# veronicaguerrini/LiME

Measured on AMD Instinct MI355X. Metric: eBWT symbols/s processed (ClusterLCP+ClusterBWT_DA), higher is better.
Workload: dtype u8

## Files before the change

include/lime_hip.h:

```cpp
#ifndef LIME_HIP_H
#define LIME_HIP_H
#include <stddef.h>
#include <stdint.h>

#ifdef __cplusplus
extern "C" {
#endif

#define LIME_OK            0
#define LIME_ERR_ARG      (-1)
#define LIME_ERR_HIP      (-2)
#define LIME_ERR_NOMEM    (-3)
#define LIME_ERR_MAXLEN   (-4)
#define LIME_ERR_HALO     (-5)
#define LIME_ERR_DOCID    (-6)
#define LIME_ERR_IO       (-7)

#define LIME_MAX_CLUSTER  65536u
#define LIME_TILE         4096u
#define LIME_FASTA_BLOCK  4096u

typedef struct lime_ctx lime_ctx;

typedef struct { uint64_t pStart, len; } lime_cluster_t;
// ... 78 lines not shown
                   const uint8_t *d_ebwt, uint64_t n_own, uint64_t n_avail, int eof,
                   uint32_t n_reads, uint32_t n_refs, uint32_t alpha,
                   uint8_t *d_sim, int zero_sim, void *stream);

typedef struct {
    uint32_t n_bins, bin_shift;
    const uint32_t *d_recs;
    const uint64_t *d_binbase;
    const uint64_t *d_bigrecs;
    uint64_t n_bigrecs;
} lime_records_t;
int lime_records_layout(lime_ctx *ctx, uint32_t n_reads, uint32_t n_refs, uint32_t *n_bins, uint32_t *bin_shift);
int lime_fused_records_dev(lime_ctx *ctx, const uint32_t *d_lcp, const uint32_t *d_da, const uint8_t *d_ebwt,
                           uint64_t n_own, uint64_t n_avail, int eof, uint32_t n_reads, uint32_t n_refs,
                           uint32_t alpha, void *stream);
int lime_records_get(lime_ctx *ctx, lime_records_t *out, uint64_t *h_binbase , void *stream);
int lime_apply_records_dev(lime_ctx *ctx, uint32_t n_src, const uint32_t *d_rx, const uint64_t *h_srcoff ,
                           uint32_t nb, uint32_t bin_shift, const uint64_t *d_bigrecs, uint64_t n_bigrecs,
                           uint64_t cell_lo, uint64_t block_bytes, uint8_t *d_block, void *stream);

int lime_partition_records_dev(lime_ctx *ctx, uint32_t n_prod, uint32_t prod_waves, uint32_t n_sub, uint32_t cap_w, const uint32_t *h_pool,
                               const uint32_t *h_wave_cnt, uint32_t n_bins, uint32_t bin_shift, uint32_t *d_out, uint64_t out_words,
                               uint64_t *h_binbase , int *kernel , void *stream);

int lime_combine_edges(const uint32_t *edge, uint32_t n_shards);

int lime_detect_dev(lime_ctx *ctx, const uint32_t *d_lcp, const uint32_t *d_da,
                    uint64_t n_own, uint64_t n_avail, int eof, uint64_t pos_base,
                    uint32_t n_reads, uint32_t alpha,
                    const lime_cluster_t **d_clusters, uint64_t *n_clusters, uint64_t *max_len,
                    void *stream);

int lime_score_dev(lime_ctx *ctx, const uint32_t *d_da, const uint8_t *d_ebwt, uint64_t n,
                   const lime_cluster_t *d_clusters, uint64_t n_clusters,
                   uint32_t n_reads, uint32_t n_refs, uint8_t *d_sim, int zero_sim, void *stream);

int lime_choose_dev(lime_ctx *ctx, const uint8_t *d_sim, uint32_t n_reads, uint32_t n_refs,
                    uint8_t *d_row_max, uint32_t *d_row_nnz, void *stream);

int lime_choose_pairs_dev(lime_ctx *ctx, const uint8_t *d_sim, uint32_t n_reads, uint32_t n_refs,
                          uint32_t norm, float beta, uint8_t *row_max, uint64_t *row_off,
                          lime_pair_t **pairs, uint64_t *n_pairs, void *stream);

int lime_fused_choose_dev(lime_ctx *ctx, const uint32_t *d_lcp, const uint32_t *d_da, const uint8_t *d_ebwt, uint64_t n,
                          uint32_t n_reads, uint32_t n_refs, uint32_t alpha, uint32_t norm, float beta,
                          uint8_t *row_max, uint64_t *row_off, lime_pair_t **pairs, uint64_t *n_pairs,
// ... 23 lines not shown
int  lime_comm_exchange_records(lime_comm *comm, lime_ctx *ctx, uint32_t n_reads, uint32_t n_refs, uint8_t *d_block,
                                size_t block_cap, uint64_t *cell_lo, uint64_t *block_bytes, void *stream);

int  lime_fused_multi(int n_dev, const int *devices, const uint32_t *lcp, const uint32_t *da, const uint8_t *ebwt,
                      uint64_t n, uint32_t n_reads, uint32_t n_refs, uint32_t alpha, uint8_t *sim,
                      uint64_t *n_clusters, uint64_t *max_len);

int  lime_score_choose_multi(int n_dev, const int *devices, const uint32_t *da, const uint8_t *ebwt, uint64_t n,
                             const lime_cluster_t *clusters, uint64_t n_clusters, uint32_t n_reads, uint32_t n_refs,
                             uint32_t norm, float beta, uint8_t *row_max, uint64_t *row_off, lime_pair_t **pairs,
                             uint64_t *n_pairs);

uint8_t lime_sym_index(uint8_t byte);
uint8_t lime_pair_score(const uint8_t cr[16], const uint8_t cg[16]);

typedef struct { uint32_t n_bins, bin_shift, n_sub, sub_rb, sub_gb; } lime_rec_layout_t;
int      lime_rec_layout(uint32_t n_reads, uint32_t n_refs, uint32_t one_level, uint32_t two_level, lime_rec_layout_t *out);
int      lime_rec_valid(uint32_t gd, uint32_t n_refs);
uint32_t lime_rec_of(uint32_t rd, uint32_t gd, uint32_t n_refs);
uint32_t lime_rec_sub2(uint32_t rd, uint32_t gd, uint32_t sub_rb, uint32_t sub_gb);
uint32_t lime_rec_bin(uint32_t rec, uint32_t sub, uint32_t bin_shift);
int      lime_rec_batch(const uint32_t *rd, const uint32_t *gd, uint64_t n, uint32_t n_refs, const lime_rec_layout_t *layout,
                        int fixed_slot, uint8_t *valid, uint8_t *stored, uint32_t *rec, uint32_t *sub, uint32_t *bin);
typedef struct { uint32_t cap, cap_short, room_left, top_left; } lime_scan_queue_t;
void     lime_scan_queue(lime_scan_queue_t *out);

int lime_write_clrs(const char *path, const lime_cluster_t *clusters, uint64_t n_clusters);
int lime_write_aux(const char *path, uint32_t n_reads, uint32_t n_refs, uint32_t alpha,
                   uint64_t max_len, uint64_t n_clusters);
int lime_read_aux(const char *path, uint32_t *n_reads, uint32_t *n_refs, uint32_t *alpha,
                  uint64_t *max_len, uint64_t *n_clusters);
int lime_write_res_txt(const char *path, const uint8_t *sim, const uint8_t *row_max,
                       uint32_t n_reads, uint32_t n_refs, uint32_t norm, float beta);
int lime_write_res_bin(const char *path_bin, const char *path_pos, const uint8_t *sim,
                       const uint8_t *row_max, uint32_t n_reads, uint32_t n_refs,
                       uint32_t norm, float beta);
int lime_write_res_txt_pairs(const char *path, const uint8_t *row_max, const uint64_t *row_off,
                             const lime_pair_t *pairs, uint32_t n_reads, uint32_t norm, float beta);
int lime_write_res_bin_pairs(const char *path_bin, const char *path_pos, const uint8_t *row_max,
                             const uint64_t *row_off, const lime_pair_t *pairs, uint32_t n_reads,
                             uint32_t norm, float beta);

int lime_classify(uint32_t n_files, const char *const *inputs, int binary, uint32_t n_reads,
                  uint32_t n_targ, const char *path_out, const char *path_tax, int rank, int higher,
                  uint64_t counts[4]);
const char *lime_classify_error(void);
// ... 168 lines not shown
```

lime_amd/_lib.py:

```python
from __future__ import annotations

import ctypes as C
import os

_DIR = os.path.dirname(os.path.abspath(__file__))
LIB_PATH = os.environ.get("LIME_LIB") or os.path.join(_DIR, "liblime_hip.so")

LIME_OK = 0
ERR_ARG, ERR_HIP, ERR_NOMEM, ERR_MAXLEN, ERR_HALO, ERR_DOCID, ERR_IO = -1, -2, -3, -4, -5, -6, -7
MAX_CLUSTER = 65536
TILE = 4096
FASTA_BLOCK = 4096


class Cluster(C.Structure):
    _fields_ = [("pStart", C.c_uint64), ("len", C.c_uint64)]


class Stats(C.Structure):
    _fields_ = [("n_clusters", C.c_uint64), ("max_len", C.c_uint64), ("n_updates", C.c_uint64),
                ("n_cross", C.c_uint32), ("n_big", C.c_uint32), ("flags", C.c_uint32), ("wave_records_max", C.c_uint32), ("edge", C.c_uint32), ("reserved", C.c_uint32)]


class Records(C.Structure):
# ... 48 lines not shown
    "lime_register_file": (_i, [_vp, _sz, _i]),
    "lime_unregister_file": (None, [_vp]),
    "lime_score": (_i, [_vp, _vp, _vp, _u64, _vp, _u64, _u32, _u32, _vp]),
    "lime_fused": (_i, [_vp, _vp, _vp, _vp, _u64, _u32, _u32, _u32, _vp, _pu64, _pu64]),
    "lime_choose": (_i, [_vp, _vp, _u32, _u32, _vp, _vp]),
    "lime_sim_bytes": (_sz, [_u32, _u32]),
    "lime_fused_dev": (_i, [_vp, _vp, _vp, _vp, _u64, _u64, _i, _u32, _u32, _u32, _vp, _i, _vp]),
    "lime_detect_dev": (_i, [_vp, _vp, _vp, _u64, _u64, _i, _u64, _u32, _u32, _pp, _pu64, _pu64, _vp]),
    "lime_score_dev": (_i, [_vp, _vp, _vp, _u64, _vp, _u64, _u32, _u32, _vp, _i, _vp]),
    "lime_choose_dev": (_i, [_vp, _vp, _u32, _u32, _vp, _vp, _vp]),
    "lime_synth_dev": (_i, [_vp, _u64, _u64, _u64, _u32, _u32, _u32, _u32, _vp, _vp, _vp, _vp]),
    "lime_get_stats": (_i, [_vp, C.POINTER(Stats), _vp]),
    "lime_set_timing": (_i, [_vp, _i]),
    "lime_get_timing": (_i, [_vp, C.POINTER(C.c_double), _pu64]),
    "lime_get_timing_ex": (_i, [_vp, C.POINTER(C.c_double), _pu64]),
    "lime_get_host_times": (_i, [_vp, C.POINTER(C.c_double)]),
    "lime_sym_index": (C.c_uint8, [C.c_uint8]),
    "lime_pair_score": (C.c_uint8, [_vp, _vp]),
    "lime_rec_layout": (_i, [_u32, _u32, _u32, _u32, _vp]),
    "lime_rec_valid": (_i, [_u32, _u32]),
    "lime_rec_of": (_u32, [_u32, _u32, _u32]),
    "lime_rec_sub2": (_u32, [_u32, _u32, _u32, _u32]),
    "lime_rec_bin": (_u32, [_u32, _u32, _u32]),
    "lime_rec_batch": (_i, [_vp, _vp, _u64, _u32, _vp, _i, _vp, _vp, _vp, _vp, _vp]),
    "lime_scan_queue": (None, [_vp]),
    "lime_write_clrs": (_i, [C.c_char_p, _vp, _u64]),
    "lime_write_aux": (_i, [C.c_char_p, _u32, _u32, _u32, _u64, _u64]),
    "lime_read_aux": (_i, [C.c_char_p, C.POINTER(_u32), C.POINTER(_u32), C.POINTER(_u32), _pu64, _pu64]),
    "lime_write_res_txt": (_i, [C.c_char_p, _vp, _vp, _u32, _u32, _u32, C.c_float]),
    "lime_write_res_bin": (_i, [C.c_char_p, C.c_char_p, _vp, _vp, _u32, _u32, _u32, C.c_float]),
    "lime_classify": (_i, [_u32, _vp, _i, _u32, _u32, C.c_char_p, C.c_char_p, _i, _i, _vp]),
    "lime_classify_error": (C.c_char_p, []),
    "lime_fused_stream": (_i, [_vp, _vp, _vp, _vp, _u64, _u32, _u32, _u32, _u64, _vp, _pu64, _pu64]),
    "lime_choose_pairs_dev": (_i, [_vp, _vp, _u32, _u32, _u32, C.c_float, _vp, _vp, _pp, _pu64, _vp]),
    "lime_fused_choose_dev": (_i, [_vp, _vp, _vp, _vp, _u64, _u32, _u32, _u32, _u32, C.c_float, _vp, _vp, _pp, _pu64, C.POINTER(Stats), _vp]),
    "lime_score_choose": (_i, [_vp, _vp, _vp, _u64, _vp, _u64, _u32, _u32, _u32, C.c_float, _vp, _vp, _pp, _pu64, _vp]),
    "lime_combine_edges": (_i, [_vp, _u32]),
    "lime_comm_unique_id": (_i, [_vp]),
    "lime_comm_init": (_i, [_vp, _i, _i, _pp]),
    "lime_comm_destroy": (None, [_vp]),
    "lime_comm_count": (_i, [_vp, C.POINTER(_i)]),
    "lime_comm_error": (C.c_char_p, []),
    "lime_comm_reduce_scatter_tables": (_i, [_vp, _vp, _vp, _sz, _vp]),
    "lime_comm_allreduce_tables": (_i, [_vp, _vp, _sz, _vp]),
    "lime_comm_combine_counters": (_i, [_vp, _vp, _vp]),
    "lime_records_layout": (_i, [_vp, _u32, _u32, C.POINTER(_u32), C.POINTER(_u32)]),
    "lime_fused_records_dev": (_i, [_vp, _vp, _vp, _vp, _u64, _u64, _i, _u32, _u32, _u32, _vp]),
    "lime_records_get": (_i, [_vp, _vp, _vp, _vp]),
    "lime_apply_records_dev": (_i, [_vp, _u32, _vp, _vp, _u32, _u32, _vp, _u64, _u64, _u64, _vp, _vp]),
    "lime_partition_records_dev": (_i, [_vp, _u32, _u32, _u32, _u32, _vp, _vp, _u32, _u32, _vp, _u64, _vp, C.POINTER(_i), _vp]),
    "lime_comm_exchange_records": (_i, [_vp, _vp, _u32, _u32, _vp, _sz, _pu64, _pu64, _vp]),
    "lime_fused_multi": (_i, [_i, _vp, _vp, _vp, _vp, _u64, _u32, _u32, _u32, _vp, _pu64, _pu64]),
    "lime_score_choose_multi": (_i, [_i, _vp, _vp, _vp, _u64, _vp, _u64, _u32, _u32, _u32, C.c_float, _vp, _vp, _pp, _pu64]),
    "lime_write_res_txt_pairs": (_i, [C.c_char_p, _vp, _vp, _vp, _u32, _u32, C.c_float]),
    "lime_write_res_bin_pairs": (_i, [C.c_char_p, C.c_char_p, _vp, _vp, _vp, _u32, _u32, C.c_float]),
    "lime_choose_lists_dev": (_i, [_vp, _vp, _u32, _u32, _u32, C.c_float, _pp, _vp]),
    "lime_fused_choose_lists_dev": (_i, [_vp, _vp, _vp, _vp, _u64, _u32, _u32, _u32, _u32, C.c_float, _pp, C.POINTER(Stats), _vp]),
    "lime_fused_choose_lists": (_i, [_vp, _vp, _vp, _vp, _u64, _u32, _u32, _u32, _u32, C.c_float, _pp, C.POINTER(Stats)]),
    "lime_lists_get": (_i, [_vp, _vp, _vp, _pp, _pu64]),
    "lime_lists_info": (_i, [_vp, C.POINTER(_u32), _pu64, C.POINTER(_u32), C.POINTER(C.c_float)]),
    "lime_lists_free": (None, [_vp]),
    "lime_lists_concat_dev": (_i, [_vp, _u32, _vp, _vp, _vp, C.c_float, _pp, _vp]),
    "lime_lists_concat_norms_dev": (_i, [_vp, _u32, _vp, _vp, _vp, _vp, C.c_float, _pp, _vp]),
    "lime_lists_get_norms": (_i, [_vp, _vp]),
    "lime_taxonomy_load": (_i, [C.c_char_p, _i, _i, _u32, _pp]),
    "lime_taxonomy_free": (None, [_vp]),
    "lime_classify_lists_dev": (_i, [_vp, _u32, _vp, _u32, _vp, _i, _vp, _vp, _vp]),
    "lime_classify_mem": (_i, [_u32, _vp, _vp, _vp, _vp, _vp, _i, _u32, _u32, _vp, _vp, _vp]),
    "lime_classify_mem_norms": (_i, [_u32, _vp, _vp, _vp, _vp, _vp, _vp, _i, _u32, _u32, _vp, _vp, _vp]),
    "lime_write_classification": (_i, [C.c_char_p, _vp, _u32]),
    "lime_index_size": (_u64, [_vp, _u32]),
    "lime_build_index": (_i, [_vp, _vp, _vp, _u32, C.c_uint8, _u32, _vp, _vp, _vp]),
# ... 114 lines not shown
```

lime_amd/api.py:

```python
from __future__ import annotations

import ctypes as C
import os

import numpy as np

from . import _lib
from ._lib import Cluster, LimeError, Stats, check, check_cls

FASTA_BLOCK = _lib.FASTA_BLOCK
NORM_PER_READ = 0xFFFFFFFF
VERDICT = np.dtype([("taxon", "<u4"), ("sim", "<f4"), ("type", "u1"), ("rule", "u1"), ("pad", "u1", (2,))])


class _LibBuf:
    def __init__(self, lib, ptr, words):
        self._lib, self._ptr = lib, ptr
        self.__array_interface__ = {"data": (ptr, False), "shape": (words,), "typestr": "<u4", "version": 3}

    def __del__(self):
        try:
            self._lib.lime_free(C.c_void_p(self._ptr))
        except Exception:
            pass
# ... 209 lines not shown
        nb, sh = C.c_uint32(0), C.c_uint32(0)
        check(self.lib.lime_records_layout(self.h, n_reads, n_refs, C.byref(nb), C.byref(sh)))
        return int(nb.value), int(sh.value)

    def fused_records_dev(self, lcp_t, da_t, ebwt_t, n_own, n_avail, eof, n_reads, n_refs, alpha, stream=None):
        self._rec_shape = self.records_layout(n_reads, n_refs)
        check(self.lib.lime_fused_records_dev(self.h, _ptr(lcp_t), _ptr(da_t), _ptr(ebwt_t), n_own, n_avail, int(eof),
                                              n_reads, n_refs, alpha, stream))

    def records_get(self, stream=None):
        import numpy as np
        from ._lib import Records
        nb, _ = self._rec_shape
        r = Records()
        base = np.zeros(nb + 1, dtype=np.uint64)
        check(self.lib.lime_records_get(self.h, C.byref(r), base.ctypes.data, stream))
        return r, base

    def apply_records_dev(self, n_src, rx_t, srcoff, nb, bin_shift, bigrecs_t, n_big, cell_lo, block_bytes, block_t, stream=None):
        import numpy as np
        so = np.ascontiguousarray(srcoff, dtype=np.uint64)
        check(self.lib.lime_apply_records_dev(self.h, n_src, _ptr(rx_t), so.ctypes.data, nb, bin_shift, _ptr(bigrecs_t), n_big,
                                              cell_lo, block_bytes, _ptr(block_t), stream))

    def partition_records(self, n_prod, prod_waves, n_sub, cap_w, pool, wave_cnt, n_bins, bin_shift, out_t, out_words=None, stream=None):
        import numpy as np
        pool = np.ascontiguousarray(pool, dtype=np.uint32)
        wc = np.ascontiguousarray(wave_cnt, dtype=np.uint32)
        base = np.zeros(n_bins + 1, dtype=np.uint64)
        kernel = C.c_int(-1)
        check(self.lib.lime_partition_records_dev(self.h, n_prod, prod_waves, n_sub, cap_w, pool.ctypes.data, wc.ctypes.data, n_bins, bin_shift,
                                                  _ptr(out_t), out_t.numel() if out_words is None else out_words, base.ctypes.data,
                                                  C.byref(kernel), stream))
        return base, int(kernel.value)

    def detect_dev(self, lcp_t, da_t, n_own, n_avail, eof, pos_base, n_reads, alpha, stream=None):
        dc, nc, ml = C.c_void_p(), C.c_uint64(0), C.c_uint64(0)
        check(self.lib.lime_detect_dev(self.h, _ptr(lcp_t), _ptr(da_t), n_own, n_avail, int(eof), pos_base, n_reads,
                                       alpha, C.byref(dc), C.byref(nc), C.byref(ml), stream))
        return dc.value, int(nc.value), int(ml.value)

    def score_dev(self, da_t, ebwt_t, n, clusters_ptr, n_clusters, n_reads, n_refs, sim_t, zero_sim=True, stream=None):
        check(self.lib.lime_score_dev(self.h, _ptr(da_t), _ptr(ebwt_t), n, C.c_void_p(clusters_ptr), n_clusters, n_reads,
                                      n_refs, _ptr(sim_t), int(zero_sim), stream))

    def choose_dev(self, sim_t, n_reads, n_refs, max_t, nnz_t, stream=None):
# ... 1126 lines not shown
```

lime_amd/csrc/lime_api.cpp:

```cpp
#include <hip/hip_runtime.h>
#include <stdarg.h>
#include <stdio.h>
#include <stdlib.h>
#include <string.h>
#include <memory>
#include <string>
#include <vector>

#include "lime_device.h"
#include "lime_ctx.h"

using namespace lime;
using namespace lime_host;

static thread_local std::string g_err;

int lime_host::fail(int code, const char *fmt, ...)
{
    char buf[512];
    va_list ap; va_start(ap, fmt); vsnprintf(buf, sizeof buf, fmt, ap); va_end(ap);
    g_err = buf;
    return code;
}

// ... 308 lines not shown

extern "C" uint8_t lime_pair_score(const uint8_t cr[16], const uint8_t cg[16])
{
    uint32_t r[4] = {0, 0, 0, 0}, g[4] = {0, 0, 0, 0};
    for (int i = 0; i < 16; ++i) { r[i >> 2] |= (uint32_t)cr[i] << ((i & 3) * 8); g[i >> 2] |= (uint32_t)cg[i] << ((i & 3) * 8); }
    return (uint8_t)pair_score(r, g);
}

extern "C" int lime_rec_layout(uint32_t n_reads, uint32_t n_refs, uint32_t one_level, uint32_t two_level, lime_rec_layout_t *out)
{
    if (!n_reads || !n_refs || !out) return fail(LIME_ERR_ARG, "lime_rec_layout: bad argument");
    const size_t sim_bytes = lime_sim_bytes(n_reads, n_refs);
    if (sim_bytes > ((size_t)BIN_MAX << BIN_SHIFT_MAX) || sim_bytes >= (1ull << CELL_BITS) || sim_bytes > ((uint64_t)MAX_SUB << 32))
        return fail(LIME_ERR_ARG, "lime_rec_layout: table too large for update records");
    const bool forced = one_level && two_level;
    bin_layout_of(forced ? one_level : BIN_ONE_LEVEL, forced ? two_level : BIN_TWO_LEVEL, forced, sim_bytes, &out->n_bins, &out->bin_shift);
    sub_layout(sim_bytes, n_refs, &out->n_sub, &out->sub_rb, &out->sub_gb);
    return LIME_OK;
}
extern "C" int lime_rec_valid(uint32_t gd, uint32_t n_refs) { return genome_ok(gd, n_refs) ? 1 : 0; }
extern "C" uint32_t lime_rec_of(uint32_t rd, uint32_t gd, uint32_t n_refs) { return rec_of(rd, gd, n_refs); }
extern "C" uint32_t lime_rec_sub2(uint32_t rd, uint32_t gd, uint32_t sub_rb, uint32_t sub_gb) { return rec_sub2(rd, gd, sub_rb, sub_gb); }
extern "C" uint32_t lime_rec_bin(uint32_t rec, uint32_t sub, uint32_t bin_shift) { return rec_bin(rec, sub, bin_shift); }
extern "C" void lime_scan_queue(lime_scan_queue_t *out)
{
    if (out) { out->cap = QCAP_SCAN; out->cap_short = QCAP_SCAN_SHORT; out->room_left = ROOM_LEFT; out->top_left = FLUSH_GRAN - 1u; }
}
extern "C" int lime_rec_batch(const uint32_t *rd, const uint32_t *gd, uint64_t n, uint32_t n_refs, const lime_rec_layout_t *lay, int fixed_slot,
                              uint8_t *valid, uint8_t *stored, uint32_t *rec, uint32_t *sub, uint32_t *bin)
{
    if (!lay || !n_refs || (n && (!rd || !gd || !valid || !stored || !rec || !sub || !bin))) return fail(LIME_ERR_ARG, "lime_rec_batch: bad argument");
    for (uint64_t i = 0; i < n; ++i) {
        valid[i] = genome_ok(gd[i], n_refs);
        stored[i] = rec_stored(rd[i], gd[i], n_refs, lay->n_sub, lay->sub_rb, lay->sub_gb, fixed_slot != 0, rec[i], sub[i]);
        bin[i] = rec_bin(rec[i], sub[i], lay->bin_shift);
    }
    return LIME_OK;
}
```

lime_amd/csrc/lime_apply.hip:

```cpp
#define LIME_DEBUG_TU_APPLY
#include <hip/hip_runtime.h>
#include <stdint.h>
#include <string.h>
#include <atomic>
#include "lime_device.h"
#include "lime_kernels.h"
#include "lime_wave.h"
#include "lime_debug.h"
#include "lime_launch.h"

namespace lime {

__device__ __forceinline__ uint32_t keep_bytes(uint32_t x, uint32_t wb, uint32_t s, uint32_t e)
{
    uint32_t m = 0xFFFFFFFFu;
    if (wb < s) { const uint32_t d = s - wb; m = d >= 4u ? 0u : m << (8u * d); }
    if (wb + 4u > e) { const uint32_t d = e > wb ? e - wb : 0u; m &= d >= 4u ? 0xFFFFFFFFu : ((1u << (8u * d)) - 1u); }
    return x & m;
}
__device__ __forceinline__ uint32_t nz_bytes(uint32_t x) { return (((x & 0x7F7F7F7Fu) + 0x7F7F7F7Fu) | x) & 0x80808080u; }

constexpr uint32_t FIN_SEGS = 258;
__device__ __forceinline__ void fin_region_store(uint32_t *seg_acc, const ApplyFin &f, uint32_t region, uint64_t r0, uint32_t o0, uint32_t nseg, uint32_t len)
{
// ... 252 lines not shown
            for (uint32_t q = cur.q + 2u * LG; __ballot(q * 4u < cur.fe); q += 2u * LG) {
                uint2 w0 = make_uint2(0u, 0u), w1 = make_uint2(0u, 0u);
                if (q * 4u < cur.fe) w0 = *reinterpret_cast<const uint2 *>(cur.src + (size_t)q * 4u);
                if ((q + 1u) * 4u < cur.fe) w1 = *reinterpret_cast<const uint2 *>(cur.src + (size_t)(q + 1u) * 4u);
                add4c(q * 4u < cur.fe, q * 4u, w0, cur.fa, cur.fe);
                add4c((q + 1u) * 4u < cur.fe, (q + 1u) * 4u, w1, cur.fa, cur.fe);
            }
        }
    };
    uint32_t region = (gridDim.x & 7u) ? blockIdx.x : (blockIdx.x & 7u) * (gridDim.x >> 3) + (blockIdx.x >> 3);
    if (region >= n_regions) return;
    uint32_t row0 = tbase[region >> bsh], n_rows = tbase[(region >> bsh) + 1u] - row0;
    uint32_t a, e;
    index_of(region, row0, n_rows, 0u, a, e);
    uint4 ri = make_uint4(0u, 0u, 0u, 0u);
    if (MODE != 0) ri = fin.region_rows[region];
    if (MODE == 1) for (uint32_t i = threadIdx.x; i < 2u * FIN_SEGS; i += APPLY_WG) seg_acc[i] = 0u;
    bool clean = false;
    __syncthreads();
    AP_DECL
    for (;;) {
        const uint32_t next = region + gridDim.x;
        const bool more = next < n_regions;
        uint32_t nrow0 = 0, nrow1 = 0;
        if (more) { nrow0 = tbase[next >> bsh]; nrow1 = tbase[(next >> bsh) + 1u]; }
        uint4 nri = make_uint4(0u, 0u, 0u, 0u);
        if (MODE != 0 && more) nri = fin.region_rows[next];
        const bool skip = MODE == 2 && (ri.w >> 31) != 0u;
        if (MODE == 1 && threadIdx.x == 0) qovf_s[par ^ 1u] = 0u;
        if (!skip)
        for (exact = false;; exact = true) {
        qn = 0u;
        if (!(MODE == 1 && clean && !exact)) {
            for (uint32_t i = threadIdx.x; i < RW / 4; i += APPLY_WG) reg4[i] = make_uint4(0u, 0u, 0u, 0u);
            __syncthreads();
        }
        AP(0)
        for (uint32_t outer = 0; outer < n_rows; outer += NWV * 64u) {
            const uint32_t nl = runs_of(n_rows, outer);
            if (outer || exact) index_of(region, row0, n_rows, outer, a, e);
            if (MODE != 0 || lg < 6u) { if (nl) grouped_runs(a, e, nl, row0 + outer + wave); continue; }
            Step nxt;
            if (nl) load_step(0u, nxt, a, e, nl, row0 + outer + wave);
            AP(1)
            for (uint32_t l0 = 0; l0 < nl; l0 += UR) {
                AP_WAITVM AP(2)
                Step cur = nxt;
                if (l0 + UR < nl) load_step(l0 + UR, nxt, a, e, nl, row0 + outer + wave);
// ... 24 lines not shown
                            if ((q + 64u) * 4u < fe) w2 = *reinterpret_cast<const uint2 *>(cur.src[u] + (size_t)(q + 64u) * 4u);
                        }
                    }
                }
                AP(4)
            }
        }
        if (MODE == 1 && qn > QW && lane == 0u) qovf_s[par] = 1u;
        __syncthreads();
        AP(5)
        if (exact || !ovf_s) break;
        __syncthreads();
        if (threadIdx.x == 0) ovf_s = 0u;
        }
        if (MODE != 0 && !skip && fin.big_off) {
            const uint64_t lo = fin.big_off[region], hi = fin.big_off[region + 1u];
            for (uint64_t i = lo + threadIdx.x; i < hi; i += APPLY_WG) {
                const uint64_t r = fin.bigrecs[i];
                add_exact((uint32_t)r & ((1u << REGION_SHIFT) - 1u), (uint32_t)(r >> CELL_BITS));
            }
            __syncthreads();
        }
        uint32_t na = 0, ne = 0;
        if (more) index_of(next, nrow0, nrow1 - nrow0, 0u, na, ne);
        if (MODE != 0) {
            if (!skip) {
                const uint32_t len = ri.w & 0x7FFFFFFFu;
                clean = false;
                const bool has_big = fin.big_off && fin.big_off[region + 1u] != fin.big_off[region];
                if (MODE == 1 && ri.z <= FIN_SEGS && fin.n_refs >= 16u && !exact && !has_big && qovf_s[par] == 0u) {
                    const uint16_t *myq = cell_q + wave * QW;
                    uint8_t *regb = reinterpret_cast<uint8_t *>(reg4);
                    const float invf = 1.0f / (float)fin.n_refs;
                    for (uint32_t i0 = 0; i0 < qn; i0 += 64u) {
                        const uint32_t i = i0 + lane;
                        if (i < qn) {
                            const uint32_t o = myq[i], val = regb[o];
                            regb[o] = 0;
                            const uint32_t x0 = ri.y + o;
                            uint32_t seg = (uint32_t)((float)x0 * invf);
                            if (seg * fin.n_refs > x0) --seg; else if ((seg + 1u) * fin.n_refs <= x0) ++seg;
                            if (val) { atomicMax(&seg_acc[seg], val); atomicAdd(&seg_acc[ri.z + seg], 1u); }
                        }
                    }
                    __syncthreads();
                    fin_region_store(seg_acc, fin, region, (uint64_t)ri.x, ri.y, ri.z, len);
// ... 184 lines not shown
```

lime_amd/csrc/lime_device.h:

```cpp
#pragma once
#include <hip/hip_runtime.h>
#include <stdint.h>

namespace lime {

#define LIME_HD __host__ __device__ __forceinline__

LIME_HD uint32_t sym_index(uint32_t b)
{
    const uint64_t LO = 0x00E90800C200B1A0ull;
    const uint64_t HI = 0x0000000507D03640ull;
    uint32_t c = b - (uint32_t)'A';
    uint64_t tab = (c < 16u) ? LO : HI;
    uint32_t v = (uint32_t)(tab >> ((c & 15u) * 4u)) & 15u;
    v = (c < 26u) ? v : 0u;
    return (b == 0u) ? 15u : v;
}

constexpr uint64_t CORR_PACKED = 0x0F7BDE3C96A58421ull;
LIME_HD uint32_t corr_set(uint32_t a) { return (uint32_t)(CORR_PACKED >> (a * 4u)) & 15u; }

LIME_HD uint32_t iupac_match(uint32_t a, uint32_t b)
{
    uint32_t ca = corr_set(a), cb = corr_set(b);
// ... 106 lines not shown

LIME_HD bool genome_ok(uint32_t gd, uint32_t n_refs) { return gd < n_refs; }
LIME_HD uint32_t rec_of(uint32_t rd, uint32_t gd, uint32_t n_refs) { return rd * n_refs + gd; }
LIME_HD uint32_t rec_sub2(uint32_t rd, uint32_t gd, uint32_t sub_rb, uint32_t sub_gb)
{
    return (rd > sub_rb || (rd == sub_rb && gd >= sub_gb)) ? 1u : 0u;
}
LIME_HD uint32_t rec_bin_off(uint32_t sub, uint32_t bin_shift) { return sub << (32u - bin_shift); }
LIME_HD uint32_t rec_bin_at(uint32_t rec, uint32_t bin_shift, uint32_t bin_off) { return (rec >> bin_shift) + bin_off; }
LIME_HD uint32_t rec_bin(uint32_t rec, uint32_t sub, uint32_t bin_shift) { return rec_bin_at(rec, bin_shift, rec_bin_off(sub, bin_shift)); }
constexpr uint32_t REC_STAND_IN = 0u;
LIME_HD uint32_t rec_or_stand_in(bool ok, uint32_t rd, uint32_t gd, uint32_t n_refs) { return ok ? rec_of(rd, gd, n_refs) : REC_STAND_IN; }
LIME_HD uint32_t entry_or_stand_in(bool ok, uint32_t gd, uint32_t t_shift) { return ok ? gd | (1u << t_shift) : 0u; }
LIME_HD uint64_t cell_of(uint32_t rd, uint32_t gd, uint32_t n_refs) { return (uint64_t)rd * n_refs + gd; }
LIME_HD uint32_t cell_sub(uint64_t cell) { return (uint32_t)(cell >> 32); }
LIME_HD uint32_t cell_bin(uint64_t cell, uint32_t bin_shift) { return (uint32_t)(cell >> bin_shift); }
LIME_HD bool rec_stored(uint32_t rd, uint32_t gd, uint32_t n_refs, uint32_t n_sub, uint32_t sub_rb, uint32_t sub_gb, bool fixed_slot,
                        uint32_t &rec, uint32_t &sub)
{
    const bool ok = genome_ok(gd, n_refs);
    rec = rec_or_stand_in(ok, rd, gd, n_refs);
    sub = !ok || n_sub == 1u ? 0u : n_sub == 2u ? rec_sub2(rd, gd, sub_rb, sub_gb) : cell_sub(cell_of(rd, gd, n_refs));
    return ok || (fixed_slot && n_sub == 1u);
}

LIME_HD uint64_t mix64(uint64_t z)
{
    z ^= z >> 30; z *= 0xBF58476D1CE4E5B9ull;
    z ^= z >> 27; z *= 0x94D049BB133111EBull;
    z ^= z >> 31; return z;
}

LIME_HD void synth_element(uint64_t seed, uint64_t i, uint32_t n_reads, uint32_t n_refs,
                           uint32_t alpha, uint32_t mode, uint32_t &l, uint32_t &d, uint32_t &s)
{
    const uint64_t PHI = 0x9E3779B97F4A7C15ull;
    const uint32_t p_run = mode ? 24904u : 26214u;
    const uint32_t p_read = mode ? 16384u : 6554u;
    uint64_t a = mix64(seed ^ (i * PHI));
    uint64_t b = mix64(a + PHI);
    uint32_t u = (uint32_t)(a & 0xFFFF), r1 = (uint32_t)((a >> 16) & 0xFFFF);
    uint32_t v = (uint32_t)((a >> 32) & 0xFFFF);
    l = (u < p_run) ? alpha + (r1 % 48u) : (alpha ? r1 % alpha : 0u);
    if (i == 0) l = 0;
    uint32_t sel = (uint32_t)(b & 0xFFFFFFFFu);
    d = (v < p_read) ? (sel % n_reads) : n_reads + (sel % n_refs);
// ... 16 lines not shown
```

lime_amd/csrc/lime_partition.hip:

```cpp
#define LIME_DEBUG_TU_PARTITION
#include <hip/hip_runtime.h>
#include <stdint.h>
#include <atomic>
#include <type_traits>
#include "lime_device.h"
#include "lime_kernels.h"
#include "lime_wave.h"
#include "lime_debug.h"
#include "lime_launch.h"

namespace lime {


template <int WG = PART_WG>
__device__ __forceinline__ void part_scan(const uint32_t *cnt, uint32_t *toff, uint32_t nb, uint32_t *wsum)
{
    const uint32_t tid = threadIdx.x, lane = tid & 63u, wave = tid >> 6;
    const uint32_t per = (nb + WG - 1u) / WG, b0 = tid * per;
    uint32_t mine = 0;
    for (uint32_t k = 0; k < per; ++k) mine += b0 + k < nb ? cnt[b0 + k] : 0u;
    const uint32_t incl = wave_incl_scan(mine);
    if (lane == 63u) wsum[wave] = incl;
    __syncthreads();
    uint32_t run = incl - mine;
// ... 501 lines not shown
            if (dr[j] != ~0u) {
                const uint32_t d = dr[j] & 0xFFFu, r = dr[j] >> 12;
                stage[toff[d] + r] = make_uint2(gcur[d] + r, val[j]);
            }
        __syncthreads();
        const uint32_t nv = toff[f2 - 1u] + cnt[f2 - 1u];
        for (uint32_t i = tid; i < nv; i += PART_WG) { const uint2 sv = stage[i]; out[lo + sv.x] = sv.y; }
        __syncthreads();
        for (uint32_t i = tid; i < f2; i += PART_WG) { gcur[i] += cnt[i]; cnt[i] = 0u; }
        __syncthreads();
    }
}

__global__ __launch_bounds__(PART_WG) void k_tile_bases(const uint64_t *binbase, uint32_t n_bins, uint32_t *tbase)
{
    __shared__ uint32_t cnt[BIN_MAX], toff[BIN_MAX];
    __shared__ uint32_t wsum[PART_WG / 64];
    for (uint32_t b = threadIdx.x; b < n_bins; b += PART_WG) cnt[b] = (uint32_t)((binbase[b + 1] - binbase[b] + PART_TILE - 1u) / PART_TILE);
    __syncthreads();
    part_scan(cnt, toff, n_bins, wsum);
    for (uint32_t b = threadIdx.x; b < n_bins; b += PART_WG) { tbase[b] = toff[b]; if (b == n_bins - 1u) tbase[n_bins] = toff[b] + cnt[b]; }
}

__global__ __launch_bounds__(PART_WG) void k_sort_tiles(const uint32_t *recs, const uint64_t *binbase, uint32_t bin_shift,
                                                        const uint32_t *tbase, uint16_t *idx, uint16_t *out16, uint32_t nt_rows)
{
    constexpr uint32_t F2MAX = 1u << (BIN_SHIFT_MAX - REGION_SHIFT);
    __shared__ uint4 stage4[PART_TILE / 8];
    __shared__ uint32_t cnt[F2MAX], toff[F2MAX];
    __shared__ uint32_t wsum[PART_WG / 64];
    uint16_t *stage = reinterpret_cast<uint16_t *>(stage4);
    const uint32_t tid = threadIdx.x;
    const uint32_t f2 = 1u << (bin_shift - REGION_SHIFT), omask = (1u << bin_shift) - 1u;
    const uint32_t rsh = f2 <= 32u ? 4u : f2 <= 64u ? 3u : f2 <= 128u ? 2u : f2 <= 256u ? 1u : 0u, nc = f2 << rsh;
    const uint32_t mycopy = (threadIdx.x & 63u) & ((1u << rsh) - 1u);
    const uint32_t bin = blockIdx.x, kq = blockIdx.y, nq = gridDim.y;
    const uint64_t lo = binbase[bin], hi = binbase[bin + 1];
    const uint32_t row0 = tbase[bin];
    uint16_t *bidx = idx + (size_t)row0 * (f2 + 1u);
    for (uint32_t i = tid; i < nc; i += PART_WG) cnt[i] = 0u;
    __syncthreads();
    const uint64_t step = (uint64_t)PART_TILE * nq, first = lo + (uint64_t)PART_TILE * kq;
    auto load_tile = [&](uint64_t t0, uint32_t (&v)[PART_PER]) {
        const uint32_t tn = hi - t0 < PART_TILE ? (uint32_t)(hi - t0) : PART_TILE;
#pragma unroll
        for (uint32_t j = 0; j < PART_PER; ++j) {
            const uint32_t i = j * PART_WG + tid;
            v[j] = i < tn ? __builtin_nontemporal_load(recs + t0 + i) : 0u;
        }
    };
    uint32_t nxt[PART_PER];
    if (first < hi) load_tile(first, nxt);
    uint32_t row = kq;
    __shared__ uint32_t nv_s;
    const uint32_t lane = tid & 63u, wave = tid >> 6;
    ST_DECL
    for (uint64_t t0 = first; t0 < hi; t0 += step, row += nq) {
        ST_WAITVM ST(0)
        uint32_t val[PART_PER], dr[PART_PER];
#pragma unroll
        for (uint32_t j = 0; j < PART_PER; ++j) {
            val[j] = nxt[j]; dr[j] = ~0u;
            if (val[j] >> bin_shift) {
                const uint32_t d = (((val[j] & omask) >> REGION_SHIFT) << rsh) | mycopy;
                dr[j] = d | (atomicAdd(&cnt[d], 1u) << 12);
            }
        }
        ST(1)
        if (t0 + step < hi) load_tile(t0 + step, nxt);
        ST(2)
        __syncthreads();
        ST(3)
        {
            static_assert(F2MAX <= PART_WG, "a region's counter per thread");
            const uint32_t c = tid < nc ? cnt[tid] : 0u;
            const uint32_t incl = wave_incl_scan(c);
            if (lane == 63u) wsum[wave] = incl;
            __syncthreads();
            uint32_t run = incl - c;
            for (uint32_t k = 0; k < wave; ++k) run += wsum[k];
            if (tid < nc) { toff[tid] = run; cnt[tid] = 0u; if (!(tid & ((1u << rsh) - 1u))) bidx[(size_t)row * (f2 + 1u) + (tid >> rsh)] = (uint16_t)run; }
            if (tid == nc - 1u) { nv_s = run + c; bidx[(size_t)row * (f2 + 1u) + f2] = (uint16_t)(run + c); }
            __syncthreads();
        }
        ST(4)
#pragma unroll
        for (uint32_t j = 0; j < PART_PER; ++j)
            if (dr[j] != ~0u) stage[toff[dr[j] & 0xFFFu] + (dr[j] >> 12)] = (uint16_t)(val[j] & ((1u << REGION_SHIFT) - 1u));
        ST(5)
        __syncthreads();
        ST(6)
        const uint32_t nv = nv_s;
        uint4 *dst = reinterpret_cast<uint4 *>(out16 + (size_t)(row0 + row) * ROW_STRIDE);
        if (nt_rows) {
            typedef uint32_t u32x4 __attribute__((ext_vector_type(4)));
            for (uint32_t i = tid; i < (nv + 7u) / 8u; i += PART_WG) { const uint4 v = stage4[i]; const u32x4 x = {v.x, v.y, v.z, v.w}; __builtin_nontemporal_store(x, reinterpret_cast<u32x4 *>(dst + i)); }
        } else
            for (uint32_t i = tid; i < (nv + 7u) / 8u; i += PART_WG) dst[i] = stage4[i];
        ST(7)
    }
    ST_END
}

__global__ __launch_bounds__(256) void k_regroup(const uint32_t *rx, const uint64_t *srcoff, uint32_t n_src, uint32_t nb,
                                                 const uint64_t *dstbase, uint32_t *dst)
{
    const uint32_t b = blockIdx.x;
    uint64_t at = dstbase[b];
    for (uint32_t s = 0; s < n_src; ++s) {
        const uint64_t lo = srcoff[(size_t)s * (nb + 1u) + b], hi = srcoff[(size_t)s * (nb + 1u) + b + 1u];
        for (uint64_t i = lo + threadIdx.x; i < hi; i += 256u) dst[at + (i - lo)] = rx[i];
        at += hi - lo;
    }
}

void launch_part(const ScanArgs &a, uint32_t n_prod, const uint64_t *binbase, uint32_t *out, hipStream_t st, bool p64, bool lines_ok)
{
    static std::atomic<bool> attr_set[MAX_DEV];
    std::atomic<bool> &set = attr_set[cur_device()];
    if (!set.load(std::memory_order_relaxed)) {
        (void)hipFuncSetAttribute(reinterpret_cast<const void *>(k_part<PART_WG, BIN_MAX, false>), hipFuncAttributeMaxDynamicSharedMemorySize, (int)(BIN_MAX * 12u));
        (void)hipFuncSetAttribute(reinterpret_cast<const void *>(k_part<PART_WG, BIN_MAX, true>), hipFuncAttributeMaxDynamicSharedMemorySize, (int)(BIN_MAX * 16u));
// ... 21 lines not shown
        hipFuncAttributes fa;
        r = 1u;
        if (hipFuncGetAttributes(&fa, kl) == hipSuccess && fa.sharedSizeBytes < 160u * 1024u) {
            const uint32_t dyn = 160u * 1024u - (uint32_t)fa.sharedSizeBytes;
            if (hipFuncSetAttribute(kl, hipFuncAttributeMaxDynamicSharedMemorySize, (int)dyn) == hipSuccess) r = dyn;
        }
        (void)hipGetLastError();
        room.store(r, std::memory_order_relaxed);
    }
    const size_t stat = 160u * 1024u - (r > 1u ? r : 0u);
    return lds_lines <= r && 2u * (lds_lines + stat + 512u) <= 160u * 1024u;
}

void launch_part2(const uint32_t *recs, const uint64_t *binbase, uint32_t n_bins, uint32_t bin_shift, uint64_t *regbase,
                  uint32_t *out, hipStream_t st)
{
    hipLaunchKernelGGL(k_part2, dim3(n_bins), dim3(PART_WG), 0, st, recs, binbase, bin_shift, regbase, out);
}

void launch_sort_tiles(const uint32_t *recs, const uint64_t *binbase, uint32_t n_bins, uint32_t bin_shift, uint32_t *tbase, uint16_t *idx, uint16_t *out16,
                       hipStream_t st, bool big_rows, bool tbase_ready)
{
    if (!tbase_ready) hipLaunchKernelGGL(k_tile_bases, dim3(1), dim3(PART_WG), 0, st, binbase, n_bins, tbase);
    const uint32_t per_bin = n_bins >= 2048u ? 1u : (2048u + n_bins - 1u) / n_bins;
    hipLaunchKernelGGL(k_sort_tiles, dim3(n_bins, per_bin), dim3(PART_WG), 0, st, recs, binbase, bin_shift, tbase, idx, out16, big_rows ? 1u : 0u);
}

uint64_t tiles_bound(uint64_t n_records, uint32_t n_bins) { return n_records / PART_TILE + n_bins; }

uint32_t part_tile() { return PART_TILE; }
uint32_t row_stride() { return ROW_STRIDE; }

void launch_regroup(const uint32_t *rx, const uint64_t *srcoff, uint32_t n_src, uint32_t nb, const uint64_t *dstbase, uint32_t *dst, hipStream_t st)
{
    if (nb) hipLaunchKernelGGL(k_regroup, dim3(nb), dim3(256), 0, st, rx, srcoff, n_src, nb, dstbase, dst);
}

void preload_partition()
{
    preload_kernel(k_part<PART_WG, BIN_MAX, false>); preload_kernel(k_part<PART_WG, BIN_MAX, true>);
    preload_kernel(k_part_lines<false>); preload_kernel(k_part_lines<true>); preload_kernel(k_tile_bases); preload_kernel(k_sort_tiles);
}

}
```

lime_amd/csrc/lime_pass.cpp:

```cpp
#include <hip/hip_runtime.h>
#include <stdio.h>
#include <string.h>
#include <chrono>
#include <string>
#include <vector>

#include "lime_device.h"
#include "lime_ctx.h"

using namespace lime;
using namespace lime_host;

static int ensure_scratch(lime_ctx *c, uint64_t n_avail, bool detect, bool score, hipStream_t st, double *acct)
{
    const size_t n_tiles = (size_t)((n_avail + WIN - 1) / WIN);
    int rc;
    const size_t have = std::min(std::min(c->summ.cap, c->tile_cnt.cap), std::min(c->tile_off.cap, c->cross.cap));
    const size_t cap = n_tiles > have ? n_tiles + 16 : have;
    if ((rc = c->summ.ensure(cap, st, acct)) || (rc = c->tile_cnt.ensure(cap, st, acct)) || (rc = c->tile_off.ensure(cap, st, acct)) ||
        (rc = c->cross.ensure(cap, st, acct))) return rc;
    if (score) {
        const uint64_t want_small = 16, want_big = n_avail / (4u * SMALL_MAX) + 65536u;
        if (want_big > 0xFFFFFFF0ull) return fail(LIME_ERR_ARG, "array too long for one shard: %llu", (unsigned long long)n_avail);
        if ((rc = c->small.ensure(want_small, st, acct)) || (rc = c->big.ensure(want_big, st, acct))) return rc;
// ... 441 lines not shown
    int rc;
    const size_t segs = (size_t)n_prod * prod_waves * n_sub, pool_words = segs * cap_w;
    if ((rc = c->pool.ensure(pool_words + 16, st, nullptr)) || (rc = ensure_bin_counters(c, segs, counts.size(), st, nullptr))) return rc;
    if (pool_words) HIP_TRY(hipMemcpyAsync(c->pool.p, h_pool, pool_words * sizeof(uint32_t), hipMemcpyHostToDevice, st));
    HIP_TRY(hipMemcpyAsync(c->wave_cnt.p, h_wave_cnt, segs * sizeof(uint32_t), hipMemcpyHostToDevice, st));
    HIP_TRY(hipMemcpyAsync(c->counts.p, counts.data(), counts.size() * sizeof(uint32_t), hipMemcpyHostToDevice, st));
    ScanArgs a;
    memset(&a, 0, sizeof a);
    a.upd_mode = 1; a.pool = c->pool.p; a.cap_w = cap_w; a.n_sub = n_sub; a.wave_cnt = c->wave_cnt.p; a.counts = c->counts.p;
    a.n_bins = n_bins; a.bin_shift = bin_shift; a.prod_waves = prod_waves;
    launch_bin_rowscan(c->counts.p, c->totals.p, n_bins, n_prod, st);
    launch_bin_bases(c->totals.p, c->binbase.p, nullptr, n_bins, st);
    uint32_t *out = d_out;
    if (c->p64_test_base) {
        launch_add_u64(c->binbase.p, (size_t)n_bins + 1, c->p64_test_base, st);
        out = d_out - c->p64_test_base;
    }
    launch_part(a, n_prod, c->binbase.p, out, st, p64, c->part_lines != 0);
    HIP_TRY(hipGetLastError());
    HIP_TRY(hipMemcpyAsync(h_binbase, c->binbase.p, ((size_t)n_bins + 1) * sizeof(uint64_t), hipMemcpyDeviceToHost, st));
    return LIME_OK;
}

extern "C" int lime_partition_records_dev(lime_ctx *c, uint32_t n_prod, uint32_t prod_waves, uint32_t n_sub, uint32_t cap_w, const uint32_t *h_pool,
                                          const uint32_t *h_wave_cnt, uint32_t n_bins, uint32_t bin_shift, uint32_t *d_out, uint64_t out_words,
                                          uint64_t *h_binbase, int *kernel, void *stream)
{
    int rc = check_ctx(c, "lime_partition_records_dev"); if (rc) return rc;
    hipStream_t st = (hipStream_t)stream;
    if (!h_pool || !h_wave_cnt || !d_out || !h_binbase || !kernel) return fail(LIME_ERR_ARG, "lime_partition_records_dev: NULL argument");
    if (!n_prod || prod_waves < 1u || prod_waves > 16u || n_sub < 1u || n_sub > MAX_SUB || (cap_w & 15u))
        return fail(LIME_ERR_ARG, "lime_partition_records_dev: want n_prod >= 1, 1 <= prod_waves <= 16, 1 <= n_sub <= %u, cap_w a multiple of 16", MAX_SUB);
    if (bin_shift < REGION_SHIFT || bin_shift > BIN_SHIFT_MAX || n_bins < 1u || n_bins > BIN_MAX)
        return fail(LIME_ERR_ARG, "lime_partition_records_dev: want %u <= bin_shift <= %u and 1 <= n_bins <= %u", REGION_SHIFT, BIN_SHIFT_MAX, BIN_MAX);
    if (misaligned(d_out, 64)) return fail(LIME_ERR_ARG, "lime_partition_records_dev: d_out must be 64-byte aligned");
    if ((uint64_t)prod_waves * n_sub * cap_w > 0xFFFFFFF0ull || (uint64_t)n_bins * n_prod > 0xFFFFFFF0ull)
        return fail(LIME_ERR_ARG, "lime_partition_records_dev: pool too large");
    const size_t segs = (size_t)n_prod * prod_waves * n_sub;
    uint64_t total = 0;
    for (size_t i = 0; i < segs; ++i) {
        if (h_wave_cnt[i] > cap_w) return fail(LIME_ERR_ARG, "lime_partition_records_dev: segment %zu holds %u records, cap_w is %u", i, h_wave_cnt[i], cap_w);
        total += h_wave_cnt[i];
    }
    if (total > out_words) return fail(LIME_ERR_ARG, "lime_partition_records_dev: %llu records, out_words is %llu", (unsigned long long)total, (unsigned long long)out_words);
    if ((c->p64_test_base + total) >> (32u + 31u - bin_shift)) return fail(LIME_ERR_ARG, "lime_partition_records_dev: positions beyond what bin_shift %u leaves room for", bin_shift);
    std::vector<uint32_t> counts((size_t)n_bins * n_prod, 0u);
// ... 153 lines not shown
```

Baseline: 336.3 billion.

## Make tile sort a persistent grid over global tile rows with prefetched lookup

The tile sort kernel stops launching one grid slice per bin and instead runs a persistent grid sized to resident blocks. Each block walks global tile rows, finding each row's bin by a distributed binary search over a shared copy of the tile bases, and looks the next tile up two iterations ahead. This aims to balance load across bins of uneven size and to remove idle blocks. In the apply kernel, the two tile-base loads become one per-lane load plus readlane. A host-side getter for the tile index is added for testing.

Result: no change. 338.9 billion (median of 6 runs) (+0.8%).

```diff
diff --git a/include/lime_hip.h b/include/lime_hip.h
--- a/include/lime_hip.h
+++ b/include/lime_hip.h
@@ -124,6 +124,7 @@
 int lime_partition_records_dev(lime_ctx *ctx, uint32_t n_prod, uint32_t prod_waves, uint32_t n_sub, uint32_t cap_w, const uint32_t *h_pool,
                                const uint32_t *h_wave_cnt, uint32_t n_bins, uint32_t bin_shift, uint32_t *d_out, uint64_t out_words,
                                uint64_t *h_binbase , int *kernel , void *stream);
+int lime_tile_index_get(lime_ctx *ctx, uint32_t n_bins, uint32_t bin_shift, uint32_t *h_tbase, uint16_t *h_idx, uint64_t idx_rows);
 
 int lime_combine_edges(const uint32_t *edge, uint32_t n_shards);
 
@@ -193,6 +194,7 @@
 uint32_t lime_rec_bin(uint32_t rec, uint32_t sub, uint32_t bin_shift);
 int      lime_rec_batch(const uint32_t *rd, const uint32_t *gd, uint64_t n, uint32_t n_refs, const lime_rec_layout_t *layout,
                         int fixed_slot, uint8_t *valid, uint8_t *stored, uint32_t *rec, uint32_t *sub, uint32_t *bin);
+uint32_t lime_tile_bin(const uint32_t *tbase, uint32_t n_bins, uint32_t row);
 typedef struct { uint32_t cap, cap_short, room_left, top_left; } lime_scan_queue_t;
 void     lime_scan_queue(lime_scan_queue_t *out);
 
diff --git a/lime_amd/_lib.py b/lime_amd/_lib.py
--- a/lime_amd/_lib.py
+++ b/lime_amd/_lib.py
@@ -94,6 +94,7 @@
     "lime_rec_of": (_u32, [_u32, _u32, _u32]),
     "lime_rec_sub2": (_u32, [_u32, _u32, _u32, _u32]),
     "lime_rec_bin": (_u32, [_u32, _u32, _u32]),
+    "lime_tile_bin": (_u32, [_vp, _u32, _u32]),
     "lime_rec_batch": (_i, [_vp, _vp, _u64, _u32, _vp, _i, _vp, _vp, _vp, _vp, _vp]),
     "lime_scan_queue": (None, [_vp]),
     "lime_write_clrs": (_i, [C.c_char_p, _vp, _u64]),
@@ -120,6 +121,7 @@
     "lime_fused_records_dev": (_i, [_vp, _vp, _vp, _vp, _u64, _u64, _i, _u32, _u32, _u32, _vp]),
     "lime_records_get": (_i, [_vp, _vp, _vp, _vp]),
     "lime_apply_records_dev": (_i, [_vp, _u32, _vp, _vp, _u32, _u32, _vp, _u64, _u64, _u64, _vp, _vp]),
+    "lime_tile_index_get": (_i, [_vp, _u32, _u32, _vp, _vp, _u64]),
     "lime_partition_records_dev": (_i, [_vp, _u32, _u32, _u32, _u32, _vp, _vp, _u32, _u32, _vp, _u64, _vp, C.POINTER(_i), _vp]),
     "lime_comm_exchange_records": (_i, [_vp, _vp, _u32, _u32, _vp, _sz, _pu64, _pu64, _vp]),
     "lime_fused_multi": (_i, [_i, _vp, _vp, _vp, _vp, _u64, _u32, _u32, _u32, _vp, _pu64, _pu64]),
diff --git a/lime_amd/api.py b/lime_amd/api.py
--- a/lime_amd/api.py
+++ b/lime_amd/api.py
@@ -255,6 +255,14 @@
         so = np.ascontiguousarray(srcoff, dtype=np.uint64)
         check(self.lib.lime_apply_records_dev(self.h, n_src, _ptr(rx_t), so.ctypes.data, nb, bin_shift, _ptr(bigrecs_t), n_big,
                                               cell_lo, block_bytes, _ptr(block_t), stream))
+
+    def tile_index(self, n_bins, bin_shift, max_rows):
+        import numpy as np
+        tbase = np.zeros(n_bins + 1, dtype=np.uint32)
+        per = (1 << (bin_shift - 16)) + 1
+        idx = np.zeros((max(int(max_rows), 1), per), dtype=np.uint16)
+        check(self.lib.lime_tile_index_get(self.h, n_bins, bin_shift, tbase.ctypes.data, idx.ctypes.data, int(max_rows)))
+        return tbase, idx[:min(int(tbase[-1]), int(max_rows))]
 
     def partition_records(self, n_prod, prod_waves, n_sub, cap_w, pool, wave_cnt, n_bins, bin_shift, out_t, out_words=None, stream=None):
         import numpy as np
diff --git a/lime_amd/csrc/lime_api.cpp b/lime_amd/csrc/lime_api.cpp
--- a/lime_amd/csrc/lime_api.cpp
+++ b/lime_amd/csrc/lime_api.cpp
@@ -354,6 +354,7 @@
 extern "C" uint32_t lime_rec_of(uint32_t rd, uint32_t gd, uint32_t n_refs) { return rec_of(rd, gd, n_refs); }
 extern "C" uint32_t lime_rec_sub2(uint32_t rd, uint32_t gd, uint32_t sub_rb, uint32_t sub_gb) { return rec_sub2(rd, gd, sub_rb, sub_gb); }
 extern "C" uint32_t lime_rec_bin(uint32_t rec, uint32_t sub, uint32_t bin_shift) { return rec_bin(rec, sub, bin_shift); }
+extern "C" uint32_t lime_tile_bin(const uint32_t *tbase, uint32_t n_bins, uint32_t row) { return tbase && n_bins ? tile_bin(tbase, n_bins, row) : 0u; }
 extern "C" void lime_scan_queue(lime_scan_queue_t *out)
 {
     if (out) { out->cap = QCAP_SCAN; out->cap_short = QCAP_SCAN_SHORT; out->room_left = ROOM_LEFT; out->top_left = FLUSH_GRAN - 1u; }
diff --git a/lime_amd/csrc/lime_apply.hip b/lime_amd/csrc/lime_apply.hip
--- a/lime_amd/csrc/lime_apply.hip
+++ b/lime_amd/csrc/lime_apply.hip
@@ -298,8 +298,8 @@
     for (;;) {
         const uint32_t next = region + gridDim.x;
         const bool more = next < n_regions;
-        uint32_t nrow0 = 0, nrow1 = 0;
-        if (more) { nrow0 = tbase[next >> bsh]; nrow1 = tbase[(next >> bsh) + 1u]; }
+        uint32_t nrv = 0;
+        if (more) nrv = tbase[(next >> bsh) + ((lane ^ par) & 1u)];
         uint4 nri = make_uint4(0u, 0u, 0u, 0u);
         if (MODE != 0 && more) nri = fin.region_rows[next];
         const bool skip = MODE == 2 && (ri.w >> 31) != 0u;
@@ -370,6 +370,7 @@
             __syncthreads();
         }
         uint32_t na = 0, ne = 0;
+        const uint32_t nrow0 = (uint32_t)__builtin_amdgcn_readlane((int)nrv, (int)par), nrow1 = (uint32_t)__builtin_amdgcn_readlane((int)nrv, (int)(par ^ 1u));
         if (more) index_of(next, nrow0, nrow1 - nrow0, 0u, na, ne);
         if (MODE != 0) {
             if (!skip) {
diff --git a/lime_amd/csrc/lime_device.h b/lime_amd/csrc/lime_device.h
--- a/lime_amd/csrc/lime_device.h
+++ b/lime_amd/csrc/lime_device.h
@@ -152,6 +152,18 @@
     rec = rec_or_stand_in(ok, rd, gd, n_refs);
     sub = !ok || n_sub == 1u ? 0u : n_sub == 2u ? rec_sub2(rd, gd, sub_rb, sub_gb) : cell_sub(cell_of(rd, gd, n_refs));
     return ok || (fixed_slot && n_sub == 1u);
+}
+
+LIME_HD uint32_t tile_bin(const uint32_t *tbase, uint32_t n_bins, uint32_t row)
+{
+    uint32_t lo = 0, n = n_bins;
+    while (n > 1u) {
+        const uint32_t half = n >> 1;
+        const bool up = tbase[lo + half] <= row;
+        lo = up ? lo + half : lo;
+        n = up ? n - half : half;
+    }
+    return lo;
 }
 
 LIME_HD uint64_t mix64(uint64_t z)
diff --git a/lime_amd/csrc/lime_partition.hip b/lime_amd/csrc/lime_partition.hip
--- a/lime_amd/csrc/lime_partition.hip
+++ b/lime_amd/csrc/lime_partition.hip
@@ -547,27 +547,43 @@
     for (uint32_t b = threadIdx.x; b < n_bins; b += PART_WG) { tbase[b] = toff[b]; if (b == n_bins - 1u) tbase[n_bins] = toff[b] + cnt[b]; }
 }
 
-__global__ __launch_bounds__(PART_WG) void k_sort_tiles(const uint32_t *recs, const uint64_t *binbase, uint32_t bin_shift,
+__global__ __launch_bounds__(PART_WG) void k_sort_tiles(const uint32_t *recs, const uint64_t *binbase, uint32_t n_bins, uint32_t bin_shift,
                                                         const uint32_t *tbase, uint16_t *idx, uint16_t *out16, uint32_t nt_rows)
 {
     constexpr uint32_t F2MAX = 1u << (BIN_SHIFT_MAX - REGION_SHIFT);
     __shared__ uint4 stage4[PART_TILE / 8];
     __shared__ uint32_t cnt[F2MAX], toff[F2MAX];
     __shared__ uint32_t wsum[PART_WG / 64];
+    __shared__ uint32_t tb_s[BIN_MAX + 1u];
+    __shared__ uint64_t bb_s[BIN_MAX + 1u];
     uint16_t *stage = reinterpret_cast<uint16_t *>(stage4);
     const uint32_t tid = threadIdx.x;
     const uint32_t f2 = 1u << (bin_shift - REGION_SHIFT), omask = (1u << bin_shift) - 1u;
     const uint32_t rsh = f2 <= 32u ? 4u : f2 <= 64u ? 3u : f2 <= 128u ? 2u : f2 <= 256u ? 1u : 0u, nc = f2 << rsh;
     const uint32_t mycopy = (threadIdx.x & 63u) & ((1u << rsh) - 1u);
-    const uint32_t bin = blockIdx.x, kq = blockIdx.y, nq = gridDim.y;
-    const uint64_t lo = binbase[bin], hi = binbase[bin + 1];
-    const uint32_t row0 = tbase[bin];
-    uint16_t *bidx = idx + (size_t)row0 * (f2 + 1u);
+    const uint32_t n_tiles = tbase[n_bins], grid = gridDim.x;
+    uint32_t row = blockIdx.x;
+    if (row >= n_tiles) return;
+    for (uint32_t i = tid; i <= n_bins; i += PART_WG) { tb_s[i] = tbase[i]; bb_s[i] = binbase[i]; }
     for (uint32_t i = tid; i < nc; i += PART_WG) cnt[i] = 0u;
     __syncthreads();
-    const uint64_t step = (uint64_t)PART_TILE * nq, first = lo + (uint64_t)PART_TILE * kq;
-    auto load_tile = [&](uint64_t t0, uint32_t (&v)[PART_PER]) {
-        const uint32_t tn = hi - t0 < PART_TILE ? (uint32_t)(hi - t0) : PART_TILE;
+    __shared__ uint64_t d_t0[2];
+    __shared__ uint32_t d_tn[2];
+    const uint32_t per = (n_bins + PART_WG - 1u) / PART_WG, b0 = tid * per, mine = b0 < n_bins ? (n_bins - b0 < per ? n_bins - b0 : per) : 0u;
+    auto find_tile = [&](uint32_t r, uint32_t slot) {
+        if (r >= n_tiles) { if (tid == 0) d_tn[slot] = 0u; return; }
+        if (mine && tb_s[b0] <= r && r < tb_s[b0 + mine]) {
+            const uint32_t b = b0 + tile_bin(tb_s + b0, mine, r);
+            const uint64_t at = bb_s[b] + (uint64_t)PART_TILE * (r - tb_s[b]), left = bb_s[b + 1u] - at;
+            d_t0[slot] = at; d_tn[slot] = left < PART_TILE ? (uint32_t)left : PART_TILE;
+        }
+    };
+    auto found_tile = [&](uint32_t slot, uint64_t &t0, uint32_t &tn) {
+        const uint64_t at = d_t0[slot];
+        tn = (uint32_t)__builtin_amdgcn_readfirstlane((int)d_tn[slot]);
+        t0 = ((uint64_t)(uint32_t)__builtin_amdgcn_readfirstlane((int)(uint32_t)(at >> 32)) << 32) | (uint32_t)__builtin_amdgcn_readfirstlane((int)(uint32_t)at);
+    };
+    auto load_tile = [&](uint64_t t0, uint32_t tn, uint32_t (&v)[PART_PER]) {
 #pragma unroll
         for (uint32_t j = 0; j < PART_PER; ++j) {
             const uint32_t i = j * PART_WG + tid;
@@ -575,12 +591,18 @@
         }
     };
     uint32_t nxt[PART_PER];
-    if (first < hi) load_tile(first, nxt);
-    uint32_t row = kq;
+    uint64_t t0n; uint32_t tnn;
+    uint32_t slot = 0;
+    find_tile(row, 0u); find_tile(row + grid, 1u);
+    __syncthreads();
+    found_tile(0u, t0n, tnn);
+    load_tile(t0n, tnn, nxt);
+    found_tile(1u, t0n, tnn);
+    __syncthreads();
     __shared__ uint32_t nv_s;
     const uint32_t lane = tid & 63u, wave = tid >> 6;
     ST_DECL
-    for (uint64_t t0 = first; t0 < hi; t0 += step, row += nq) {
+    for (;; row += grid) {
         ST_WAITVM ST(0)
         uint32_t val[PART_PER], dr[PART_PER];
 #pragma unroll
@@ -592,9 +614,12 @@
             }
         }
         ST(1)
-        if (t0 + step < hi) load_tile(t0 + step, nxt);
+        const bool more = tnn != 0u;
+        if (more) load_tile(t0n, tnn, nxt);
+        find_tile(row + 2u * grid, slot);
         ST(2)
         __syncthreads();
+        found_tile(slot, t0n, tnn); slot ^= 1u;
         ST(3)
         {
             static_assert(F2MAX <= PART_WG, "a region's counter per thread");
@@ -604,8 +629,8 @@
             __syncthreads();
             uint32_t run = incl - c;
             for (uint32_t k = 0; k < wave; ++k) run += wsum[k];
-            if (tid < nc) { toff[tid] = run; cnt[tid] = 0u; if (!(tid & ((1u << rsh) - 1u))) bidx[(size_t)row * (f2 + 1u) + (tid >> rsh)] = (uint16_t)run; }
-            if (tid == nc - 1u) { nv_s = run + c; bidx[(size_t)row * (f2 + 1u) + f2] = (uint16_t)(run + c); }
+            if (tid < nc) { toff[tid] = run; cnt[tid] = 0u; if (!(tid & ((1u << rsh) - 1u))) idx[(size_t)row * (f2 + 1u) + (tid >> rsh)] = (uint16_t)run; }
+            if (tid == nc - 1u) { nv_s = run + c; idx[(size_t)row * (f2 + 1u) + f2] = (uint16_t)(run + c); }
             __syncthreads();
         }
         ST(4)
@@ -616,13 +641,14 @@
         __syncthreads();
         ST(6)
         const uint32_t nv = nv_s;
-        uint4 *dst = reinterpret_cast<uint4 *>(out16 + (size_t)(row0 + row) * ROW_STRIDE);
+        uint4 *dst = reinterpret_cast<uint4 *>(out16 + (size_t)row * ROW_STRIDE);
         if (nt_rows) {
             typedef uint32_t u32x4 __attribute__((ext_vector_type(4)));
             for (uint32_t i = tid; i < (nv + 7u) / 8u; i += PART_WG) { const uint4 v = stage4[i]; const u32x4 x = {v.x, v.y, v.z, v.w}; __builtin_nontemporal_store(x, reinterpret_cast<u32x4 *>(dst + i)); }
         } else
             for (uint32_t i = tid; i < (nv + 7u) / 8u; i += PART_WG) dst[i] = stage4[i];
         ST(7)
+        if (!more) break;
     }
     ST_END
 }
@@ -690,8 +716,11 @@
                        hipStream_t st, bool big_rows, bool tbase_ready)
 {
     if (!tbase_ready) hipLaunchKernelGGL(k_tile_bases, dim3(1), dim3(PART_WG), 0, st, binbase, n_bins, tbase);
-    const uint32_t per_bin = n_bins >= 2048u ? 1u : (2048u + n_bins - 1u) / n_bins;
-    hipLaunchKernelGGL(k_sort_tiles, dim3(n_bins, per_bin), dim3(PART_WG), 0, st, recs, binbase, bin_shift, tbase, idx, out16, big_rows ? 1u : 0u);
+    static std::atomic<uint32_t> resident_of[MAX_DEV];
+    std::atomic<uint32_t> &slot = resident_of[cur_device()];
+    uint32_t resident = slot.load(std::memory_order_relaxed);
+    if (!resident) { resident = resident_blocks(k_sort_tiles, PART_WG); slot.store(resident, std::memory_order_relaxed); }
+    if (n_bins) hipLaunchKernelGGL(k_sort_tiles, dim3(resident), dim3(PART_WG), 0, st, recs, binbase, n_bins, bin_shift, tbase, idx, out16, big_rows ? 1u : 0u);
 }
 
 uint64_t tiles_bound(uint64_t n_records, uint32_t n_bins) { return n_records / PART_TILE + n_bins; }
diff --git a/lime_amd/csrc/lime_pass.cpp b/lime_amd/csrc/lime_pass.cpp
--- a/lime_amd/csrc/lime_pass.cpp
+++ b/lime_amd/csrc/lime_pass.cpp
@@ -487,6 +487,20 @@
     return LIME_OK;
 }
 
+extern "C" int lime_tile_index_get(lime_ctx *c, uint32_t n_bins, uint32_t bin_shift, uint32_t *h_tbase, uint16_t *h_idx, uint64_t idx_rows)
+{
+    int rc = check_ctx(c, "lime_tile_index_get"); if (rc) return rc;
+    if (!h_tbase || !h_idx || n_bins < 1u || n_bins > BIN_MAX || bin_shift <= REGION_SHIFT || bin_shift > BIN_SHIFT_MAX || !c->tbase.p || !c->tidx.p)
+        return fail(LIME_ERR_ARG, "lime_tile_index_get: bad argument, or no second level by tiles has run");
+    HIP_TRY(hipDeviceSynchronize());
+    HIP_TRY(hipMemcpy(h_tbase, c->tbase.p, ((size_t)n_bins + 1) * sizeof(uint32_t), hipMemcpyDeviceToHost));
+    const size_t per = ((size_t)1 << (bin_shift - REGION_SHIFT)) + 1u;
+    size_t rows = h_tbase[n_bins] < idx_rows ? h_tbase[n_bins] : (size_t)idx_rows;
+    if (rows * per > c->tidx.cap) rows = c->tidx.cap / per;
+    if (rows) HIP_TRY(hipMemcpy(h_idx, c->tidx.p, rows * per * sizeof(uint16_t), hipMemcpyDeviceToHost));
+    return LIME_OK;
+}
+
 extern "C" int lime_partition_records_dev(lime_ctx *c, uint32_t n_prod, uint32_t prod_waves, uint32_t n_sub, uint32_t cap_w, const uint32_t *h_pool,
                                           const uint32_t *h_wave_cnt, uint32_t n_bins, uint32_t bin_shift, uint32_t *d_out, uint64_t out_words,
                                           uint64_t *h_binbase, int *kernel, void *stream)
```
